# paTRICK-swk/D3DP

Measured on AMD Instinct MI355X. Metric: pose-hypotheses/sec (H x clips) at F=243, J=17, H=20, K=10, higher is better.
Workload: dtype f16x2-split operands on fp16 MFMA, f32 accumulate (fp32-class: meets 1e-3 mm)

## Files before the change

### d3dp_amd/csrc/attention_x2.hip

```cpp
#include "common.h"
#include "kernels.h"
#include "ta_common.h"
#include "attn_frag.h"

#ifndef D3DP_ATTN_OVERLAP
#define D3DP_ATTN_OVERLAP 0
#endif
#ifndef D3DP_ATTN_KPIPE
#define D3DP_ATTN_KPIPE 0
#endif
#ifndef D3DP_ATTN_MIXLO
#define D3DP_ATTN_MIXLO 0
#endif
#ifndef D3DP_ATTN_W16
#define D3DP_ATTN_W16 0
#endif
#ifndef D3DP_ATTN_STAMP
#define D3DP_ATTN_STAMP 0
#endif

namespace {

__device__ __forceinline__ f16x8 as_f16x8(bf16x8 v) { return __builtin_bit_cast(f16x8, v); }

// ... 30 lines not shown
#pragma unroll
  for (int dn = 0; dn < ND; ++dn) o[dn] = __builtin_amdgcn_mfma_f32_16x16x32_f16(vh[dn], pl[C0], o[dn], 0, 0, 0);
#pragma unroll
  for (int dn = 0; dn < ND; ++dn) o[dn] = __builtin_amdgcn_mfma_f32_16x16x32_f16(vh[dn], ph[C0], o[dn], 0, 0, 0);
  __builtin_amdgcn_sched_barrier(0);
  if constexpr (C0 + 1 < C1) pv_chunks_x2_rec<NKT, C0 + 1, C1>(fb, plane, ph, pl, o, nh, nl);
}
template <int NKT, int C0, int C1 = NKT / 2, int HD>
__device__ __forceinline__ void pv_chunks_x2(const FragBasesT<HD>& fb, int plane, const f16x8 (&ph)[NKT / 2],
                                             const f16x8 (&pl)[NKT / 2], f32x4 (&o)[HD / 16]) {
  if constexpr (C0 < C1) {
    f16x8 vh[HD / 16], vl[HD / 16];
    load_v_frags_x2<C0>(fb, plane, vh, vl);
    pv_chunks_x2_rec<NKT, C0, C1>(fb, plane, ph, pl, o, vh, vl);
  }
}

template <int C0, int HD>
__device__ __forceinline__ void pv_chunk_x2_seq(const FragBasesT<HD>& fb, int plane, const f16x8& ph, const f16x8& pl,
                                                f32x4 (&o)[HD / 16]) {
#pragma unroll
  for (int dn = 0; dn < HD / 16; ++dn) {
    const f16x8 vh = load_vt_frag<C0, f16, HD>(fb.v[dn]);
    const f16x8 vl = load_vt_frag<C0, f16, HD>(fb.v[dn] + plane);
    o[dn] = __builtin_amdgcn_mfma_f32_16x16x32_f16(vl, ph, o[dn], 0, 0, 0);
    o[dn] = __builtin_amdgcn_mfma_f32_16x16x32_f16(vh, pl, o[dn], 0, 0, 0);
    o[dn] = __builtin_amdgcn_mfma_f32_16x16x32_f16(vh, ph, o[dn], 0, 0, 0);
  }
}

// ... 74 lines not shown
  asm volatile("global_load_dwordx4 %0, %1, off" : "=v"(r) : "v"(p) : "memory");
  return r;
}
__device__ __forceinline__ void settle(f32x4& r) { asm volatile("" : "+v"(r)); }
__device__ __forceinline__ void gload16_untracked_into(f32x4& r, const float* p) {
  asm volatile("global_load_dwordx4 %0, %1, off" : "+v"(r) : "v"(p) : "memory");
}

template <int V>
__device__ __forceinline__ void wait_vmcnt() { __builtin_amdgcn_s_waitcnt((V & 15) | (7 << 4) | (15 << 8) | ((V >> 4) << 14)); }

#if D3DP_ATTN_OVERLAP || D3DP_ATTN_MIXLO || D3DP_ATTN_W16
#include "attention_x2_variants.h"
#endif

template <int NKT, bool MASK_ANY_TILE>
__device__ __forceinline__ void softmax_split_x2(f32x4 (&s)[NKT], int n, int lane, f16x8 (&ph)[NKT / 2], f16x8 (&pl)[NKT / 2],
                                                 float& denom, float cexp) {
  const int fg = lane >> 4;
  if constexpr (!MASK_ANY_TILE) {
#pragma unroll
    for (int r = 0; r < 4; ++r)
      if (16 * (NKT - 1) + 4 * fg + r >= n) s[NKT - 1][r] = -INFINITY;
  } else {
#pragma unroll
    for (int t = 0; t < NKT; ++t)
#pragma unroll
      for (int r = 0; r < 4; ++r)
        if (16 * t + 4 * fg + r >= n) s[t][r] = -INFINITY;
  }
  float mx = -INFINITY;
// ... 15 lines not shown
      const float y0 = __builtin_amdgcn_exp2f(fmaf(s[t][r], cexp, nb)), y1 = __builtin_amdgcn_exp2f(fmaf(s[t][r + 1], cexp, nb));
      sum4[0] += y0;
      sum4[1] += y1;
      const f16x2v h2 = {(f16)y0, (f16)y1};
      hp[r >> 1] = __builtin_bit_cast(unsigned, h2);
      lp[r >> 1] = x2_lo_pair_mix(y0, y1, hp[r >> 1]);
    }
    using u32x4v = unsigned __attribute__((ext_vector_type(4)));
    u32x4v hv = __builtin_bit_cast(u32x4v, ph[t >> 1]), lv = __builtin_bit_cast(u32x4v, pl[t >> 1]);
    hv[(t & 1) * 2] = hp[0]; hv[(t & 1) * 2 + 1] = hp[1];
    lv[(t & 1) * 2] = lp[0]; lv[(t & 1) * 2 + 1] = lp[1];
    ph[t >> 1] = __builtin_bit_cast(f16x8, hv);
    pl[t >> 1] = __builtin_bit_cast(f16x8, lv);
  }
#else
#pragma unroll
  for (int t = 0; t < NKT; ++t) {
#pragma unroll
    for (int r = 0; r < 4; ++r) {
      const float y = __builtin_amdgcn_exp2f(fmaf(s[t][r], cexp, nb));
      sum4[r & 1] += y;
      const f16 h = (f16)y;
      ph[t >> 1][(t & 1) * 4 + r] = h;
      pl[t >> 1][(t & 1) * 4 + r] = (f16)fmaf(y, 1.0f, -(float)h);
    }
  }
#endif
  float sum = sum4[0] + sum4[1];
  sum += __shfl_xor(sum, 16, 64);
  sum += __shfl_xor(sum, 32, 64);
// ... 39 lines not shown
    b = __builtin_amdgcn_mfma_f32_16x16x32_f16(kc[1][3], qh[1], b, 0, 0, 0);
    s[t] = a; s[t + 1] = b;
    if (t + 2 < NKT) {
#pragma unroll
      for (int j = 0; j < 2; ++j) {
        kc[j][0] = kn[j][0]; kc[j][1] = kn[j][1];
        kc[j][2] = *reinterpret_cast<const f16x8*>(fb.k0 + (t + 2 + j) * 2048);
        kc[j][3] = *reinterpret_cast<const f16x8*>(fb.k1 + (t + 2 + j) * 2048);
      }
    }
    __builtin_amdgcn_sched_barrier(0);
  }
  softmax_split_x2<NKT, MASK_ANY_TILE>(s, n, lane, ph, pl, denom, cexp);
}

template <int NKT, bool MASK_ANY_TILE>
__device__ __forceinline__ void attn_scores_x2_pair(const FragBases& fb, int plane, const f16x8 (&qh)[2][2],
                                                    const f16x8 (&ql)[2][2], int n, int lane, f16x8 (&ph)[2][NKT / 2],
                                                    f16x8 (&pl)[2][NKT / 2], float (&denom)[2], float cexp) {
  f32x4 s0[NKT], s1[NKT];
  auto read_k = [&](int t, f16x8 (&k)[4]) {
    k[0] = *reinterpret_cast<const f16x8*>(fb.k0 + plane + t * 2048);
    k[1] = *reinterpret_cast<const f16x8*>(fb.k1 + plane + t * 2048);
    k[2] = *reinterpret_cast<const f16x8*>(fb.k0 + t * 2048);
    k[3] = *reinterpret_cast<const f16x8*>(fb.k1 + t * 2048);
  };
  f16x8 kc[2][4];
#define X2_PAIR_TERM(KI, Q, D)                                                                  \
    a0 = __builtin_amdgcn_mfma_f32_16x16x32_f16(kc[0][KI], Q[0][D], a0, 0, 0, 0);               \
    b0 = __builtin_amdgcn_mfma_f32_16x16x32_f16(kc[1][KI], Q[0][D], b0, 0, 0, 0);               \
    a1 = __builtin_amdgcn_mfma_f32_16x16x32_f16(kc[0][KI], Q[1][D], a1, 0, 0, 0);               \
// ... 24 lines not shown
    if (t + 2 < NKT) { read_lo(t + 2, kc[0]); read_lo(t + 3, kc[1]); }
    __builtin_amdgcn_sched_barrier(0);
#endif
    X2_PAIR_TERM(2, ql, 0)
    X2_PAIR_TERM(3, ql, 1)
    X2_PAIR_TERM(2, qh, 0)
    X2_PAIR_TERM(3, qh, 1)
#if D3DP_ATTN_KPIPE
    __builtin_amdgcn_sched_barrier(0);
    if (t + 2 < NKT) { read_hi(t + 2, kc[0]); read_hi(t + 3, kc[1]); }
    __builtin_amdgcn_sched_barrier(0);
#endif
    s0[t] = a0; s0[t + 1] = b0; s1[t] = a1; s1[t + 1] = b1;
  }
#undef X2_PAIR_TERM
  softmax_split_x2<NKT, MASK_ANY_TILE>(s0, n, lane, ph[0], pl[0], denom[0], cexp);
  softmax_split_x2<NKT, MASK_ANY_TILE>(s1, n, lane, ph[1], pl[1], denom[1], cexp);
}

template <int HD, int NKT, bool MASK_ANY_TILE>
__device__ __forceinline__ void attn_scores_x2_hd(const FragBasesT<HD>& fb, int plane, const typename X2Head<HD>::frag& qh,
                                                  const typename X2Head<HD>::frag& ql, int n, int lane, f16x8 (&ph)[NKT / 2],
                                                  f16x8 (&pl)[NKT / 2], float& denom, float cexp) {
  typedef typename X2Head<HD>::frag frag;
  constexpr int TILE = 16 * X2Head<HD>::ROWB;
  f32x4 s[NKT];
#pragma unroll
  for (int t = 0; t < NKT; ++t) {
    const frag kl = *reinterpret_cast<const frag*>(fb.k0 + plane + t * TILE);
    const frag kh = *reinterpret_cast<const frag*>(fb.k0 + t * TILE);
    s[t] = x2_tile_scores(kh, kl, qh, ql);
    if ((t & 3) == 3) __builtin_amdgcn_sched_barrier(0);
// ... 27 lines not shown
  }
  softmax_split_x2<NKT, MASK_ANY_TILE>(s0, n, lane, ph[0], pl[0], denom[0], cexp);
  softmax_split_x2<NKT, MASK_ANY_TILE>(s1, n, lane, ph[1], pl[1], denom[1], cexp);
}

#if D3DP_ATTN_STAMP
__device__ unsigned long long d3dp_attn_stamps[4 * 8 * 16 * 8];
#define ATTN_STAMP(k)                                                                                          \
  do {                                                                                                         \
    if (blockIdx.x < 4 && iter < 16 && lane == 0)                                                              \
      d3dp_attn_stamps[((blockIdx.x * 8 + wave) * 16 + iter) * 8 + (k)] = __builtin_readcyclecounter();        \
  } while (0)
#else
#define ATTN_STAMP(k) do { } while (0)
#endif
template <int NKT, int OUTS, bool MASK_ANY_TILE, int HD = 64>
__global__ __launch_bounds__(512) void attn_temporal_x2_kernel(const float* __restrict__ qkv, void* __restrict__ out_v,
                                                               SeqMap map, int C, int heads, size_t plane_elems,
                                                               int n_prob, X2Scales sc) {
  using H = X2Head<HD>;
  constexpr int NW = 8;
  constexpr int TPW = (NKT + NW - 1) / NW;
  constexpr int NK = 16 * NKT;
  constexpr int PLANE = NK * H::ROWB;
  constexpr int NPC = PLANE / 1024;
  constexpr int PER = (NPC + NW - 1) / NW;
  constexpr int ND = HD / 16;
  __shared__ __attribute__((aligned(16))) char kimg[2 * PLANE];
  __shared__ __attribute__((aligned(16))) char vimg[2 * PLANE];
  const int n = map.n_tok;
  const int tid = threadIdx.x, lane = tid & 63;
// ... 116 lines not shown
        }
      }
    } else if constexpr (TPW == 2) {
      f16x8 qh[2][2], ql[2][2];
#pragma unroll
      for (int u = 0; u < 2; ++u) {
        float4 qf[4];
#pragma unroll
        for (int i = 0; i < 4; ++i) {
          settle(qr[u][i]);
          qf[i] = make_float4(qr[u][i][0], qr[u][i][1], qr[u][i][2], qr[u][i][3]);
        }
        ta_split8(qf[0], qf[1], qh[u][0], ql[u][0], sc.q);
        ta_split8(qf[2], qf[3], qh[u][1], ql[u][1], sc.q);
      }
      attn_scores_x2_pair<NKT, MASK_ANY_TILE>(fbk, PLANE, qh, ql, n, lane, ph, pl, denom, sc.cexp);
    } else {
      denom[0] = 1.f;
      if (wave < n_qt) {
        f16x8 qh[2], ql[2];
        float4 qf[4];
#pragma unroll
        for (int i = 0; i < 4; ++i) {
          settle(qr[0][i]);
          qf[i] = make_float4(qr[0][i][0], qr[0][i][1], qr[0][i][2], qr[0][i][3]);
        }
        ta_split8(qf[0], qf[1], qh[0], ql[0], sc.q);
        ta_split8(qf[2], qf[3], qh[1], ql[1], sc.q);
        attn_scores_x2<NKT, MASK_ANY_TILE>(fbk, PLANE, qh, ql, n, lane, ph[0], pl[0], denom[0], sc.cexp);
      }
    }
// ... 14 lines not shown
    const FragBasesT<HD> fb = make_frag_bases<HD>(kimg, vimg, opaque(lane));
#if D3DP_ATTN_OVERLAP
    if constexpr (OVL) {
      f32x4 o[4];
#pragma unroll
      for (int dn = 0; dn < 4; ++dn) o[dn] = (f32x4){0.f, 0.f, 0.f, 0.f};
      float sum1[2] = {0.f, 0.f};
      x2_pv_overlap<NKT>(fb, PLANE, ph[0], pl[0], o, s1, nb1, sc.cexp, ph[1], pl[1], sum1);
      denom[1] = x2_denominator(sum1);
      const int l = opaque(lane);
      const int q = wave * 16 + (l & 15);
      if (q < n)
        store_o_x2<OUTS>(o, inv_scale / denom[0], out_v, (size_t)(tok0 + q * ts), C, head * 64 + (l >> 4) * 4, sc.oplane);
    }
#endif
#pragma unroll
    for (int u = OVL ? 1 : 0; u < TPW; ++u) {
      if (u == TPW - 1 && (has_next || HD != 64)) load_q_raw(row0_n, head_n);
      const int qt = wave + u * NW;
      if (qt < n_qt) {
        f32x4 o[ND];
#pragma unroll
        for (int dn = 0; dn < ND; ++dn) o[dn] = (f32x4){0.f, 0.f, 0.f, 0.f};
        pv_chunks_x2<NKT, 0>(fb, PLANE, ph[u], pl[u], o);
        const int l = opaque(lane);
        const int q = qt * 16 + (l & 15);
        if (q < n)
          store_o_x2<OUTS>(o, inv_scale / denom[u], out_v, (size_t)(tok0 + q * ts), C, head * HD + (l >> 4) * 4, sc.oplane);
      }
    }
    if (!has_next) break;
    asm volatile("s_waitcnt lgkmcnt(0)" ::: "memory");
// ... 279 lines not shown
  }
}

template <typename K>
int x2_resident_per_cu(K kern, int threads, int at_most) {
  int nb = 0;
  if (hipOccupancyMaxActiveBlocksPerMultiprocessor(&nb, reinterpret_cast<const void*>(kern), threads, 0) != hipSuccess) {
    (void)hipGetLastError();
    return at_most;
  }
  return nb < 1 ? 1 : nb < at_most ? nb : at_most;
}

template <int NKT, int OUTS, int HD>
int launch_temporal_x2(const void* qkv, void* out, int n_seq, SeqMap map, int C, int heads, size_t plane, X2Scales sc,
                       hipStream_t st) {
  constexpr int NK = 16 * NKT;
  const size_t lds = (size_t)NK * X2Head<HD>::ROWB * 4;
  constexpr int NW = 8;
  const bool last_only = map.n_tok > 16 * (NKT - 1);
  auto kern = last_only ? attn_temporal_x2_kernel<NKT, OUTS, false, HD> : attn_temporal_x2_kernel<NKT, OUTS, true, HD>;
  static PerDeviceOnce once[2];
  const int n_wg = once[HD == 64 || last_only].get([&](int dev) {
    int per_cu = (int)((160 * 1024) / lds) < 2048 / (NW * 64) ? (int)((160 * 1024) / lds) : 2048 / (NW * 64);
    if constexpr (HD != 64) per_cu = x2_resident_per_cu(kern, NW * 64, per_cu);
    const int cus = d3dp_cu_count(dev);
    return cus < 0 ? cus : cus * per_cu;
  });
  if (n_wg < 0) return -3;
  const int n_prob = n_seq * heads;
#if D3DP_ATTN_W16
  if constexpr (NKT == 16 && HD == 64) {
    if (map.n_tok > 16 * (NKT - 1)) {
      hipLaunchKernelGGL((attn_temporal_x2_w16_kernel<OUTS>), dim3(n_prob < n_wg ? n_prob : n_wg), dim3(1024), 0, st,
                         (const float*)qkv, out, map, C, heads, plane, n_prob, sc);
      return 0;
    }
  }
#endif
  hipLaunchKernelGGL(kern, dim3(n_prob < n_wg ? n_prob : n_wg), dim3(NW * 64), 0, st, (const float*)qkv, out, map, C,
                     heads, plane, n_prob, sc);
  return 0;
}

template <int HD>
int launch_attn_x2_hd(int act, int axis, const void* qkv, void* out, int n_seq, SeqMap map, int C, int heads, float act_scale,
                      hipStream_t st, int hd_true) {
  const size_t plane = (size_t)n_seq * map.n_tok * C;
  const int n = map.n_tok;
  const float rsq = hd_true > 0 && hd_true != HD ? (float)(1.0 / sqrt((double)hd_true))
                                                 : (HD == 64 ? 0.125f : HD == 32 ? 0.17677669529663689f : 0.25f);
  const X2Scales sc = {act_scale, rsq * 1.44269504088896340736f / (act_scale * act_scale),
                       1.0f / act_scale, act_scale};
  if (axis == 0 && n <= 32) {
    const int n_prob = n_seq * heads;
    if (act == 3) hipLaunchKernelGGL((attn_spatial_x2_kernel<2, HD>), dim3((n_prob + 3) / 4), dim3(256), 0, st, (const float*)qkv, out, n_prob, map, C, heads, plane, sc);
    else hipLaunchKernelGGL((attn_spatial_x2_kernel<0, HD>), dim3((n_prob + 3) / 4), dim3(256), 0, st, (const float*)qkv, out, n_prob, map, C, heads, plane, sc);
    return 0;
  }
  if (n > 256) {
    const int groups = ((n + 15) / 16 + 7) / 8, n_work = n_seq * heads * groups;
    static PerDeviceOnce once[2];
    const int wgs = once[act == 3].get([&](int dev) {
      const int cus = d3dp_cu_count(dev);
      int per_cu = 2;
      if constexpr (HD != 64)
        per_cu = act == 3 ? x2_resident_per_cu(attn_temporal_x2_long_kernel<2, HD>, 512, 4) : x2_resident_per_cu(attn_temporal_x2_long_kernel<0, HD>, 512, 4);
      return cus < 0 ? cus : cus * per_cu;
    });
    if (wgs < 0) return -3;
    const dim3 grid(n_work < wgs ? n_work : wgs), blk(512);
    if (act == 3) hipLaunchKernelGGL((attn_temporal_x2_long_kernel<2, HD>), grid, blk, 0, st, (const float*)qkv, out, map, C, heads, groups, n_work, sc);
    else hipLaunchKernelGGL((attn_temporal_x2_long_kernel<0, HD>), grid, blk, 0, st, (const float*)qkv, out, map, C, heads, groups, n_work, sc);
    return 0;
  }
#define X2_CASE(NKT_)                                                                                         \
  return act == 3 ? launch_temporal_x2<NKT_, 2, HD>(qkv, out, n_seq, map, C, heads, plane, sc, st)            \
                  : launch_temporal_x2<NKT_, 0, HD>(qkv, out, n_seq, map, C, heads, plane, sc, st);
  if (n <= 32) { X2_CASE(2) }
  if (n <= 64) { X2_CASE(4) }
  if (n <= 128) { X2_CASE(8) }
  X2_CASE(16)
#undef X2_CASE
}

}

void d3dp_launch_qkv_pack_x2(const float* src, void* dst, size_t T, int C, float act_scale, hipStream_t st) {
  const size_t total = T * (size_t)(3 * C / 4);
  const unsigned blocks = (unsigned)((total + 255) / 256 < 8192 ? (total + 255) / 256 : 8192);
  hipLaunchKernelGGL(qkv_pack_x2_kernel, dim3(blocks ? blocks : 1), dim3(256), 0, st, src, (char*)dst, T, C, act_scale);
}

int d3dp_launch_attn_x2(int act, int axis, const void* qkv, void* out, int n_seq, SeqMap map, int C, int heads,
                        float act_scale, hipStream_t st, int hd_true) {
  if (heads < 1 || C % heads || map.n_tok < 1 || (act != 0 && act != 3) || !(act_scale > 0.f) || hd_true < 0 || hd_true > C / heads) return -2;
  switch (C / heads) {
    case 64: return launch_attn_x2_hd<64>(act, axis, qkv, out, n_seq, map, C, heads, act_scale, st, hd_true);
    case 32: return launch_attn_x2_hd<32>(act, axis, qkv, out, n_seq, map, C, heads, act_scale, st, hd_true);
    case 16: return launch_attn_x2_hd<16>(act, axis, qkv, out, n_seq, map, C, heads, act_scale, st, hd_true);
  }
  return -2;
}

#if D3DP_ATTN_STAMP
extern "C" __attribute__((visibility("default"))) int d3dp_debug_attn_stamps(unsigned long long* dst) {
  return (int)hipMemcpyFromSymbol(dst, HIP_SYMBOL(d3dp_attn_stamps), sizeof(unsigned long long) * 4 * 8 * 16 * 8);
}
#endif
```

### d3dp_amd/csrc/capi_denoise.hip

```cpp
#include "ctx.h"

AttnRoute attn_route(int mode, int exact_impl, int hd, int frames, int joints, bool long_rows, int axis) {
  const bool fast = mode == D3DP_MODE_FAST || mode == D3DP_MODE_FAST16, exact = mode == D3DP_MODE_EXACT;
  const bool mfma = hd == 64 || (mfma_head_dim(hd) && !long_rows);
  if (exact && exact_impl == 0 && mfma && (hd != 64 || frames <= 256 || !long_rows)) return AttnRoute::X2;
  if (fast && mfma) {
    if (axis == 0 && joints <= 32) return AttnRoute::FAST_SPATIAL;
    if (axis == 0 ? !long_rows : (frames <= 256 || !long_rows)) return AttnRoute::FAST_WHOLE_SEQ;
  }
  if (axis == 1 && exact && hd == 64 && frames <= 256) return AttnRoute::F32_TEMPORAL;
  return AttnRoute::ROWS;
}

namespace {

struct InferLayout {
  size_t temb, x, y1, y, bufA, bufB, lnst, ln_rowstat, nstat, total;
  InferLayout(const d3dp_ctx* c, int B, int H) {
    const d3dp_cfg& g = c->cfg;
    const size_t Tc = (size_t)std::min(c->chunk(), B * H) * c->seq_pitch(), C = g.channels, Cp = c->cp();
    size_t off = 0;
    auto take = [&](size_t bytes) { const size_t o = off; off += align_up(bytes); return o; };
    temb = take((size_t)B * C * 4);
    x = take(Tc * C * 4);
// ... 30 lines not shown
  Scope s(c, cls, st);
  return d3dp_linear_stream_scaled(epi, A, W, bias, out, M, N, K, st, ldexpf(1.f, r_in - r_out), ldexpf(1.f, -r_out), ldexpf(1.f, r_out));
}

int attention(d3dp_ctx* c, int axis, const void* qkv, void* out, int n_bh, float s_kv, hipStream_t st, int r_qkv = 0) {
  const d3dp_cfg& g = c->cfg;
  Scope s(c, axis == 0 ? P_ATTN_S : P_ATTN_T, st);
  const int n = axis == 0 ? n_bh * g.frames : n_bh * g.joints, act = c->act(), C = c->attn_cols();
  const SeqMap map = axis == 0 ? spatial_map(g.frames, g.joints, c->seq_pitch()) : temporal_map(g.frames, g.joints, c->seq_pitch());
  if (r_qkv != 0) {
    const AttnRoute r = c->route(axis);
    if (r != AttnRoute::FAST_SPATIAL && r != AttnRoute::FAST_WHOLE_SEQ) return -2;
    return d3dp_attn_fast_scaled(r == AttnRoute::FAST_SPATIAL ? 0 : 1, qkv, out, n, map, C, g.heads, st, ldexpf(1.f, 2 * r_qkv));
  }
  switch (c->route(axis)) {
    case AttnRoute::X2: return d3dp_launch_attn_x2(3, axis, qkv, out, n, map, C, g.heads, s_kv, st, g.channels / g.heads);
    case AttnRoute::FAST_SPATIAL: return d3dp_launch_attn_spatial_bf16(qkv, out, n, map, C, g.heads, st, c->fast_f16, g.channels / g.heads);
    case AttnRoute::FAST_WHOLE_SEQ: return d3dp_launch_attn_temporal_bf16(qkv, out, n, map, C, g.heads, st, c->fast_f16, g.channels / g.heads);
    case AttnRoute::F32_TEMPORAL: return d3dp_launch_attn_temporal_f32(act, qkv, out, n, map, C, g.heads, st);
    case AttnRoute::ROWS: break;
  }
  return d3dp_launch_attn_rows(act, qkv, out, n, map, C, g.heads, st);
}

int run_block(d3dp_ctx* c, const BlockDev& w, int axis, float* x, void* y1, void* y, void* bufA, void* bufB, float* slices,
              float* rowstat, int n_bh, hipStream_t st, float* nstat = nullptr) {
  const d3dp_cfg& g = c->cfg;
  const int Tc = n_bh * c->seq_pitch(), C = g.channels, Ca = c->attn_cols();
  const float s_o = c->x2_attn() ? w.s_kv : kActScale;
  if (w.r_qkv | w.r_proj | w.r_h | w.r_fc2) {
    LAUNCH_TRY(linear_f16(c, P_QKV, EPI_BIAS, 0, w.r_qkv, bufA, w.qkv_w, w.qkv_b, bufB, Tc, 3 * Ca, C, st));
// ... 121 lines not shown
```

### d3dp_amd/csrc/capi_ops.hip

```cpp
#include "ctx.h"

extern "C" {

int d3dp_debug_train_linear(const float* A, const float* W, const float* bias, float* out, int32_t M, int32_t N, int32_t K,
                            int32_t tail, unsigned* amax_out, int32_t amax_pos, void* stream) {
  if (!A || !W || !out || M < 1 || N < 4 || N % 4 || K < 32 || K % 32) return d3dp_fail(D3DP_EINVAL, "d3dp_debug_train_linear: bad argument");
  if (tail & ~17) return d3dp_fail(D3DP_EINVAL, "d3dp_debug_train_linear: tail = %d (bit 0: remainder rows as 16 x 64 blocks, bit 4: one pass)", tail);
  const int passes = (tail & 16) ? 1 : 3;
  tail &= 1;
  hipStream_t st = (hipStream_t)stream;
  char* buf = nullptr;
  const size_t a_bytes = (size_t)M * K * 4, w_bytes = (size_t)N * K * 4;
  HIP_TRY(hipMalloc((void**)&buf, a_bytes + w_bytes + 64));
  unsigned* amax = reinterpret_cast<unsigned*>(buf + a_bytes + w_bytes);
  float* uns = reinterpret_cast<float*>(amax + 8);
  int rc = hipMemsetAsync(amax, 0, 64, st) == hipSuccess ? 0 : -3;
  if (!rc) {
    d3dp_launch_absmax(A, (size_t)M * K, amax, st);
    d3dp_launch_absmax(W, (size_t)N * K, amax + 1, st);
    d3dp_launch_split2_dyn(A, buf, M, K, K, amax, uns, st);
    d3dp_launch_split2_dyn(W, buf + a_bytes, N, K, K, amax + 1, uns + 1, st);
    rc = d3dp_launch_linear_f16x2_dyn(buf, buf + a_bytes, bias, uns, uns + 1, out, M, N, K, 1, st, amax_out, amax_pos, tail, passes);
  }
  const hipError_t e = hipStreamSynchronize(st);
// ... 79 lines not shown
                       heads > 0 ? C / heads : 0);
    if (axis == 0 && J > 256) return d3dp_fail(D3DP_ENOTSUP, "MFMA spatial attention takes up to 256 joints; J=%d", J);
    if (axis == 0) LAUNCH_TRY(d3dp_attn_fast_scaled(J <= 32 ? 0 : 1, qkv, out, n_bh * F, spatial_map(F, J), C, heads, st, ldexpf(1.f, 2 * s)));
    else LAUNCH_TRY(d3dp_attn_fast_scaled(1, qkv, out, n_bh * J, temporal_map(F, J), C, heads, st, ldexpf(1.f, 2 * s)));
    HIP_TRY(hipGetLastError());
    return D3DP_OK;
  }
  const int hd_true = (impl & 255) == 1 ? impl >> 8 : 0;
  if (hd_true) {
    impl = 1;
    const int hdp = heads > 0 && C % heads == 0 ? C / heads : 0;
    if (!act_bf16 || !((hdp == 32 && hd_true == 24) || (hdp == 64 && (hd_true == 40 || hd_true == 48 || hd_true == 56))))
      return d3dp_fail(D3DP_ENOTSUP, "impl 1 | (true head dim << 8) takes 2-byte rows of head dim 32 holding 24 or 64 holding 40 / 48 / 56; C=%d "
                                "heads=%d true head dim %d is not one", C, heads, hd_true);
  }
  if (impl == 2) {
    if (act_bf16) return d3dp_fail(D3DP_EINVAL, "split-fp16 attention takes fp32 activations");
    if (heads < 1 || C % heads || !mfma_head_dim(C / heads))
      return d3dp_fail(D3DP_ENOTSUP, "impl 2 (split-fp16 attention) takes head dims 64, 32 and 16; C=%d heads=%d is head dim %d (the row "
                                "kernel, impl 0, takes it)", C, heads, heads > 0 ? C / heads : 0);
    void* packed = nullptr;
    const size_t T = (size_t)n_bh * F * J;
    HIP_TRY(hipMallocAsync(&packed, T * 12 * (size_t)C, st));
    d3dp_launch_qkv_pack_x2((const float*)qkv, packed, T, C, kActScale, st);
    const int rc = d3dp_launch_attn_x2(0, axis, packed, out, axis == 0 ? n_bh * F : n_bh * J,
                                       axis == 0 ? spatial_map(F, J) : temporal_map(F, J), C, heads, kActScale, st);
    HIP_TRY(hipFreeAsync(packed, st));
    LAUNCH_TRY(rc);
  } else if (impl == 1 && act_bf16 && (heads < 1 || C % heads || !mfma_head_dim(C / heads))) {
    return d3dp_fail(D3DP_ENOTSUP, "impl 1 on 2-byte rows takes head dims 64, 32 and 16; C=%d heads=%d is head dim %d (the row kernel, "
                              "impl 0, takes it)", C, heads, heads > 0 ? C / heads : 0);
  } else if (axis == 0 && impl == 1) {
    if (!act_bf16) return d3dp_fail(D3DP_EINVAL, "MFMA spatial attention needs bf16 activations");
    if (J <= 32) LAUNCH_TRY(d3dp_launch_attn_spatial_bf16(qkv, out, n_bh * F, spatial_map(F, J), C, heads, st, f16, hd_true));
    else if (J > 256) return d3dp_fail(D3DP_ENOTSUP, "MFMA spatial attention takes up to 256 joints; J=%d", J);
    else LAUNCH_TRY(d3dp_launch_attn_temporal_bf16(qkv, out, n_bh * F, spatial_map(F, J), C, heads, st, f16, hd_true));
  } else if (axis == 0) LAUNCH_TRY(d3dp_launch_attn_rows(act_bf16, qkv, out, n_bh * F, spatial_map(F, J), C, heads, st));
  else if (impl == 1 && !act_bf16) {
    LAUNCH_TRY(d3dp_launch_attn_temporal_f32(0, qkv, out, n_bh * J, temporal_map(F, J), C, heads, st));
  } else if (impl == 1) {
    if (!act_bf16) return d3dp_fail(D3DP_EINVAL, "MFMA temporal attention needs bf16 activations");
// ... 23 lines not shown
```

### d3dp_amd/csrc/ctx_plan.h

```cpp
#pragma once
#include <algorithm>
#include <cstdlib>
#include <cstring>

#include "../../include/d3dp_hip.h"

int d3dp_fail(int code, const char* fmt, ...) __attribute__((format(printf, 2, 3)));

struct CtxEnv {
  const char *exact_impl = nullptr, *long_attn = nullptr, *no_fold = nullptr, *defer_norm = nullptr, *train_impl = nullptr,
             *train_overlap = nullptr, *train_gelu = nullptr, *train_wgrad = nullptr, *train_ln_operand = nullptr, *train_tail = nullptr,
             *train_attn = nullptr, *train_passes = nullptr, *fast_impl = nullptr, *fast16_range = nullptr, *x2_skew = nullptr,
             *x2_pp = nullptr, *x2_wide = nullptr, *seq_pad = nullptr, *fold_ln = nullptr, *train_long_attn = nullptr;
  static CtxEnv from_process() {
    CtxEnv e;
    e.exact_impl = getenv("D3DP_EXACT_IMPL");
    e.long_attn = getenv("D3DP_LONG_ATTN");
    e.no_fold = getenv("D3DP_NO_FOLD");
    e.defer_norm = getenv("D3DP_DEFER_NORM");
    e.train_impl = getenv("D3DP_TRAIN_IMPL");
    e.train_overlap = getenv("D3DP_TRAIN_OVERLAP");
    e.train_gelu = getenv("D3DP_TRAIN_GELU");
    e.train_wgrad = getenv("D3DP_TRAIN_WGRAD");
    e.train_ln_operand = getenv("D3DP_TRAIN_LN_OPERAND");
    e.train_tail = getenv("D3DP_TRAIN_TAIL");
    e.train_attn = getenv("D3DP_TRAIN_ATTN");
    e.train_passes = getenv("D3DP_TRAIN_PASSES");
    e.fast_impl = getenv("D3DP_FAST_IMPL");
    e.fast16_range = getenv("D3DP_FAST16_RANGE");
    e.x2_skew = getenv("D3DP_X2_SKEW");
    e.x2_pp = getenv("D3DP_X2_PP");
    e.x2_wide = getenv("D3DP_X2_WIDE");
    e.seq_pad = getenv("D3DP_SEQ_PAD");
    e.fold_ln = getenv("D3DP_FOLD_LN");
    e.train_long_attn = getenv("D3DP_TRAIN_LONG_ATTN");
    return e;
  }
};

struct CtxPlan {
  int hdp = 0;
  bool fast16_scale = false;
  int train_passes = 3;
  int exact_impl_req = 0;
  bool long_rows = false;
  bool fold = true;
  bool defer = true;
  bool train_x2 = true;
  bool train_overlap = true;
  int train_overlap_sets = 2;
  bool train_gelu_in_prep = true;
  bool train_wgrad_merged = true;
  bool train_ln_direct = true;
  bool train_tail_blocks = true;
  int train_attn_x2 = 2;
  bool train_long_attn = false;
  int skew_d = 0;
  int pingpong = 0;
  int pad_override = -1;
  bool fold_ln_on = false;
};

inline bool env_is(const char* v, const char* s) { return v && !strcmp(v, s); }
inline int env_digit(const char* v, const char* allowed, int dflt) {
  return v && v[0] && !v[1] && strchr(allowed, v[0]) ? v[0] - '0' : dflt;
}
inline bool mfma_head_dim(int hd) { return hd == 64 || hd == 32 || hd == 16; }

inline bool instantiated_width(const d3dp_cfg& g) {
  const int hd = g.channels / g.heads;
  return (g.channels == 64 || g.channels == 128 || g.channels == 256 || g.channels == 512) &&
         (hd == 8 || hd == 16 || hd == 32 || hd == 64) && g.hidden >= 64 && g.hidden % 64 == 0;
}
inline bool optin_width(int c) { return c == 192 || c == 320 || c == 384 || c == 448; }
inline int padded_head_dim(int hd) { return hd <= 32 ? 32 : 64; }
inline bool x2_optin_shape(const d3dp_cfg& g) {
  const int hd = g.channels / g.heads;
  return optin_width(g.channels) && hd % 8 == 0 && hd <= 64 && g.hidden >= 64 && g.hidden % 64 == 0;
}
inline bool fast_optin_shape(const d3dp_cfg& g) {
  const int hd = g.channels / g.heads;
// ... 79 lines not shown
                                "{64,128,256,512} with head dim in {8,16,32,64} and hidden a multiple of 64; other widths run in D3DP_MODE_EXACT / "
                                "D3DP_MODE_TRAIN (fp32 implementation)",
                  g.channels, g.heads, g.hidden);
    if (g.channels > 1024 || g.channels % 4 || hd % 4 || hd > 128 || g.hidden < 4 || g.hidden % 4)
      return d3dp_fail(D3DP_ENOTSUP, "channels=%d heads=%d hidden=%d: the fp32 implementation takes channels <= 1024, head dim a multiple of 4 up to 128 "
                                "and hidden a multiple of 4", g.channels, g.heads, g.hidden);
    const int nmax = std::max(g.frames, g.joints), cap = hd <= 16 ? 16 : hd <= 32 ? 32 : hd <= 64 ? 64 : 128;
    if (train && !train_widths && !p.train_long_attn && (nmax > 256 || (size_t)nmax * (8 * (cap + 4) + 12) > 160 * 1024))
      return d3dp_fail(D3DP_ENOTSUP, "channels=%d heads=%d frames=%d joints=%d: training at a width outside {64,128,256,512} runs the fp32 attention "
                                "backward, which holds a whole sequence in LDS (<= 256 tokens; <= 153 at head dims above 64)",
                  g.channels, g.heads, g.frames, g.joints);
  }
  const bool train_f32 = env_is(e.train_impl, "f32");
  p.fold = !(e.no_fold && e.no_fold[0] == '1');
  p.defer = !(e.defer_norm && e.defer_norm[0] == '0');
  p.train_x2 = !train_f32 && (width_inst || train_widths);
  p.train_overlap = !(e.train_overlap && e.train_overlap[0] == '0');
  p.train_overlap_sets = (e.train_overlap && e.train_overlap[0] == '1') ? 1 : 2;
  p.train_gelu_in_prep = !env_is(e.train_gelu, "pass");
  p.train_wgrad_merged = !env_is(e.train_wgrad, "each");
  p.train_ln_direct = !env_is(e.train_ln_operand, "pass");
  p.train_tail_blocks = !env_is(e.train_tail, "split");
  p.train_attn_x2 = env_is(e.train_attn, "f32") ? 0 : env_is(e.train_attn, "x2t") ? 1 : 2;
  const bool superseded = !p.train_gelu_in_prep || !p.train_wgrad_merged || !p.train_tail_blocks || !p.train_ln_direct;
  if (train && e.train_passes) {
    if (strcmp(e.train_passes, "1") && strcmp(e.train_passes, "3"))
      return d3dp_fail(D3DP_ENOTSUP, "D3DP_TRAIN_PASSES=%.32s: the values a TRAIN context takes are D3DP_TRAIN_PASSES=1 (one fp16-MFMA pass per "
                                "product of the split-fp16 training Linears) and 3 (the default)", e.train_passes);
    if (e.train_passes[0] == '1') {
      if (!train_linears_split(p, g))
// ... 29 lines not shown
```

### d3dp_amd/csrc/kernels.h

```cpp
#pragma once
#include <hip/hip_runtime.h>
#include <stdint.h>

#include <mutex>

#include "train_plan.h"

struct PerDeviceOnce {
  static constexpr int kMaxDev = 64;
  std::mutex mu;
  int val[kMaxDev] = {0};
  template <class F> int get(F&& fn) {
    int dev = 0;
    if (hipGetDevice(&dev) != hipSuccess || dev < 0 || dev >= kMaxDev) return -3;
    std::lock_guard<std::mutex> lock(mu);
    if (val[dev] <= 0) {
      const int v = fn(dev);
      if (v <= 0) return v < 0 ? v : -3;
      val[dev] = v;
    }
    return val[dev];
  }
};
inline int d3dp_cu_count(int dev) {
// ... 72 lines not shown
                           int K, hipStream_t st);

struct SeqMap { int n_tok, inner, outer_stride, inner_stride, tok_stride; };
int d3dp_launch_attn_rows(int act_bf16, const void* qkv, void* out, int n_seq, SeqMap map, int C, int heads,
                          hipStream_t st, unsigned* amax = nullptr);
int d3dp_launch_attn_temporal_f32(int act, const void* qkv, void* out, int n_seq, SeqMap map, int C, int heads,
                                  hipStream_t st);
int d3dp_launch_attn_temporal_bf16(const void* qkv, void* out, int n_seq, SeqMap map, int C, int heads,
                                   hipStream_t st, int f16 = 0, int hd_true = 0);
int d3dp_launch_attn_spatial_bf16(const void* qkv, void* out, int n_seq, SeqMap map, int C, int heads, hipStream_t st,
                                  int f16 = 0, int hd_true = 0);
int d3dp_attn_fast_padded(int axis, const void* qkv, void* out, int n_seq, SeqMap map, int C, int heads, hipStream_t st, int f16,
                          int hd_true);
int d3dp_attn_fast_scaled(int axis, const void* qkv, void* out, int n_seq, SeqMap map, int C, int heads, hipStream_t st, float emul);
int d3dp_launch_attn_x2(int act, int axis, const void* qkv, void* out, int n_seq, SeqMap map, int C, int heads,
                        float act_scale, hipStream_t st, int hd_true = 0);
void d3dp_launch_qkv_pack_x2(const float* src, void* dst, size_t T, int C, float act_scale, hipStream_t st);

int d3dp_launch_time_mlp(const int64_t* t, const float* freq, const float* w1, const float* b1, const float* w2,
                         const float* b2, float* temb, int B, int C, hipStream_t st);
int d3dp_launch_embed_ln(int act_bf16, const float* x2d, const float* x3d, const float* temb, const float* ew,
                         const float* eb, const float* spos, const float* lnw, const float* lnb, float eps, float* x,
                         void* xn, int seq0, int n_seq, int H, int F, int J, int C, hipStream_t st, int SP = 0);
int d3dp_launch_ln(int act_bf16, float* x, const void* yadd, int write_x, const float* w, const float* b, float eps,
                   void* xn, int T, int C, hipStream_t st);
int d3dp_launch_ln2(int act_bf16, float* x, const void* yadd0, const void* yadd, const float* wa, const float* ba, const float* pos,
                    const float* wb, const float* bb, float eps, void* xn, int T, int C, int F, int J, hipStream_t st,
                    int SP = 0);
int d3dp_launch_ln2_defer(int act_bf16, const float* x, const float* wa, const float* ba, const float* wb, const float* bb, float eps,
                          void* xn, float* stat, int T, int C, hipStream_t st);
int d3dp_rows2_embed_ln(int act, const float* x2d, const float* x3d, const float* temb, const float* ew, const float* eb,
// ... 103 lines not shown
```

Baseline: 51.21.

## Share V fragments across two query tiles in temporal x2 attention PV

Adds a VSHARE path for the temporal split-fp16 attention kernel (HD=64, NKT=16). It computes PV for both of a wave's query tiles at once, in two head-dim halves, so each loaded V fragment feeds MFMAs for both tiles instead of being reloaded per tile. It also adds a v_fma_mix based computation of the low-half softmax residual. The path is on by default and can be turned off with an env var; it costs extra template instantiations and higher accumulator register pressure in the shared loop.

```diff
diff --git a/d3dp_amd/csrc/attention_x2.hip b/d3dp_amd/csrc/attention_x2.hip
--- a/d3dp_amd/csrc/attention_x2.hip
+++ b/d3dp_amd/csrc/attention_x2.hip
@@ -68,6 +68,44 @@
     load_v_frags_x2<C0>(fb, plane, vh, vl);
     pv_chunks_x2_rec<NKT, C0, C1>(fb, plane, ph, pl, o, vh, vl);
   }
+}
+
+template <int C0, int DN0>
+__device__ __forceinline__ void load_v_frags_x2_half(const FragBases& fb, int plane, f16x8 (&vh)[2], f16x8 (&vl)[2]) {
+#pragma unroll
+  for (int d = 0; d < 2; ++d) {
+    vh[d] = load_vt_frag<C0, f16, 64>(fb.v[DN0 + d]);
+    vl[d] = load_vt_frag<C0, f16, 64>(fb.v[DN0 + d] + plane);
+  }
+}
+template <int NKT, int DN0, int C0>
+__device__ __forceinline__ void pv_half_x2_rec(const FragBases& fb, int plane, const f16x8 (&ph)[2][NKT / 2],
+                                               const f16x8 (&pl)[2][NKT / 2], f32x4 (&o)[2][2], const f16x8 (&vh)[2],
+                                               const f16x8 (&vl)[2]) {
+  f16x8 nh[2], nl[2];
+  if constexpr (C0 + 1 < NKT / 2) load_v_frags_x2_half<C0 + 1, DN0>(fb, plane, nh, nl);
+  __builtin_amdgcn_sched_barrier(0);
+#pragma unroll
+  for (int d = 0; d < 2; ++d)
+#pragma unroll
+    for (int u = 0; u < 2; ++u) o[u][d] = __builtin_amdgcn_mfma_f32_16x16x32_f16(vl[d], ph[u][C0], o[u][d], 0, 0, 0);
+#pragma unroll
+  for (int d = 0; d < 2; ++d)
+#pragma unroll
+    for (int u = 0; u < 2; ++u) o[u][d] = __builtin_amdgcn_mfma_f32_16x16x32_f16(vh[d], pl[u][C0], o[u][d], 0, 0, 0);
+#pragma unroll
+  for (int d = 0; d < 2; ++d)
+#pragma unroll
+    for (int u = 0; u < 2; ++u) o[u][d] = __builtin_amdgcn_mfma_f32_16x16x32_f16(vh[d], ph[u][C0], o[u][d], 0, 0, 0);
+  __builtin_amdgcn_sched_barrier(0);
+  if constexpr (C0 + 1 < NKT / 2) pv_half_x2_rec<NKT, DN0, C0 + 1>(fb, plane, ph, pl, o, nh, nl);
+}
+template <int NKT, int DN0>
+__device__ __forceinline__ void pv_half_x2(const FragBases& fb, int plane, const f16x8 (&ph)[2][NKT / 2],
+                                           const f16x8 (&pl)[2][NKT / 2], f32x4 (&o)[2][2]) {
+  f16x8 vh[2], vl[2];
+  load_v_frags_x2_half<0, DN0>(fb, plane, vh, vl);
+  pv_half_x2_rec<NKT, DN0, 0>(fb, plane, ph, pl, o, vh, vl);
 }
 
 template <int C0, int HD>
@@ -172,7 +210,17 @@
 #include "attention_x2_variants.h"
 #endif
 
-template <int NKT, bool MASK_ANY_TILE>
+__device__ __forceinline__ unsigned x2_lo_pair_f32mix(float y0, float y1, unsigned hp) {
+  unsigned lp;
+  float t;
+  asm("v_fma_mix_f32 %0, %2, 1.0, -%4 op_sel_hi:[0,0,1]\n\t"
+      "v_fma_mix_f32 %1, %3, 1.0, -%4 op_sel:[0,0,1] op_sel_hi:[0,0,1]\n\t"
+      "v_cvt_pk_f16_f32 %0, %0, %1"
+      : "=&v"(lp), "=&v"(t) : "v"(y0), "v"(y1), "v"(hp));
+  return lp;
+}
+
+template <int NKT, bool MASK_ANY_TILE, bool LO_MIX = false>
 __device__ __forceinline__ void softmax_split_x2(f32x4 (&s)[NKT], int n, int lane, f16x8 (&ph)[NKT / 2], f16x8 (&pl)[NKT / 2],
                                                  float& denom, float cexp) {
   const int fg = lane >> 4;
@@ -218,6 +266,28 @@
     pl[t >> 1] = __builtin_bit_cast(f16x8, lv);
   }
 #else
+  if constexpr (LO_MIX) {
+    using f16x2v = _Float16 __attribute__((ext_vector_type(2)));
+    using f32x2v = float __attribute__((ext_vector_type(2)));
+    using u32x4v = unsigned __attribute__((ext_vector_type(4)));
+#pragma unroll
+    for (int t = 0; t < NKT; ++t) {
+      unsigned hp[2], lp[2];
+#pragma unroll
+      for (int r = 0; r < 4; r += 2) {
+        const float y0 = __builtin_amdgcn_exp2f(fmaf(s[t][r], cexp, nb)), y1 = __builtin_amdgcn_exp2f(fmaf(s[t][r + 1], cexp, nb));
+        sum4[0] += y0;
+        sum4[1] += y1;
+        hp[r >> 1] = __builtin_bit_cast(unsigned, __builtin_convertvector((f32x2v){y0, y1}, f16x2v));
+        lp[r >> 1] = x2_lo_pair_f32mix(y0, y1, hp[r >> 1]);
+      }
+      u32x4v hv = __builtin_bit_cast(u32x4v, ph[t >> 1]), lv = __builtin_bit_cast(u32x4v, pl[t >> 1]);
+      hv[(t & 1) * 2] = hp[0]; hv[(t & 1) * 2 + 1] = hp[1];
+      lv[(t & 1) * 2] = lp[0]; lv[(t & 1) * 2 + 1] = lp[1];
+      ph[t >> 1] = __builtin_bit_cast(f16x8, hv);
+      pl[t >> 1] = __builtin_bit_cast(f16x8, lv);
+    }
+  } else
 #pragma unroll
   for (int t = 0; t < NKT; ++t) {
 #pragma unroll
@@ -287,7 +357,7 @@
   softmax_split_x2<NKT, MASK_ANY_TILE>(s, n, lane, ph, pl, denom, cexp);
 }
 
-template <int NKT, bool MASK_ANY_TILE>
+template <int NKT, bool MASK_ANY_TILE, bool LO_MIX = false>
 __device__ __forceinline__ void attn_scores_x2_pair(const FragBases& fb, int plane, const f16x8 (&qh)[2][2],
                                                     const f16x8 (&ql)[2][2], int n, int lane, f16x8 (&ph)[2][NKT / 2],
                                                     f16x8 (&pl)[2][NKT / 2], float (&denom)[2], float cexp) {
@@ -342,8 +412,8 @@
     s0[t] = a0; s0[t + 1] = b0; s1[t] = a1; s1[t + 1] = b1;
   }
 #undef X2_PAIR_TERM
-  softmax_split_x2<NKT, MASK_ANY_TILE>(s0, n, lane, ph[0], pl[0], denom[0], cexp);
-  softmax_split_x2<NKT, MASK_ANY_TILE>(s1, n, lane, ph[1], pl[1], denom[1], cexp);
+  softmax_split_x2<NKT, MASK_ANY_TILE, LO_MIX>(s0, n, lane, ph[0], pl[0], denom[0], cexp);
+  softmax_split_x2<NKT, MASK_ANY_TILE, LO_MIX>(s1, n, lane, ph[1], pl[1], denom[1], cexp);
 }
 
 template <int HD, int NKT, bool MASK_ANY_TILE>
@@ -401,7 +471,7 @@
 #else
 #define ATTN_STAMP(k) do { } while (0)
 #endif
-template <int NKT, int OUTS, bool MASK_ANY_TILE, int HD = 64>
+template <int NKT, int OUTS, bool MASK_ANY_TILE, int HD = 64, bool VSHARE = false>
 __global__ __launch_bounds__(512) void attn_temporal_x2_kernel(const float* __restrict__ qkv, void* __restrict__ out_v,
                                                                SeqMap map, int C, int heads, size_t plane_elems,
                                                                int n_prob, X2Scales sc) {
@@ -548,7 +618,7 @@
         ta_split8(qf[0], qf[1], qh[u][0], ql[u][0], sc.q);
         ta_split8(qf[2], qf[3], qh[u][1], ql[u][1], sc.q);
       }
-      attn_scores_x2_pair<NKT, MASK_ANY_TILE>(fbk, PLANE, qh, ql, n, lane, ph, pl, denom, sc.cexp);
+      attn_scores_x2_pair<NKT, MASK_ANY_TILE, VSHARE && !D3DP_ATTN_MIXLO>(fbk, PLANE, qh, ql, n, lane, ph, pl, denom, sc.cexp);
     } else {
       denom[0] = 1.f;
       if (wave < n_qt) {
@@ -593,8 +663,30 @@
         store_o_x2<OUTS>(o, inv_scale / denom[0], out_v, (size_t)(tok0 + q * ts), C, head * 64 + (l >> 4) * 4, sc.oplane);
     }
 #endif
-#pragma unroll
-    for (int u = OVL ? 1 : 0; u < TPW; ++u) {
+    constexpr bool SHARE = VSHARE && HD == 64 && TPW == 2 && !OVL;
+    if constexpr (SHARE) {
+      const int l = opaque(lane);
+      const int q0 = wave * 16 + (l & 15);
+      const bool tile1 = wave + NW < n_qt;
+      const float inv[2] = {inv_scale / denom[0], inv_scale / denom[1]};
+#pragma unroll
+      for (int half = 0; half < 2; ++half) {
+        if (half == 1 && has_next) load_q_raw(row0_n, head_n);
+        f32x4 o[2][2];
+#pragma unroll
+        for (int u = 0; u < 2; ++u)
+#pragma unroll
+          for (int d = 0; d < 2; ++d) o[u][d] = (f32x4){0.f, 0.f, 0.f, 0.f};
+        if (half == 0) pv_half_x2<NKT, 0>(fb, PLANE, ph, pl, o);
+        else pv_half_x2<NKT, 2>(fb, PLANE, ph, pl, o);
+        const int col = head * 64 + half * 32 + (l >> 4) * 4;
+        if (q0 < n) store_o_x2<OUTS>(o[0], inv[0], out_v, (size_t)(tok0 + q0 * ts), C, col, sc.oplane);
+        if (tile1 && q0 + 16 * NW < n)
+          store_o_x2<OUTS>(o[1], inv[1], out_v, (size_t)(tok0 + (q0 + 16 * NW) * ts), C, col, sc.oplane);
+      }
+    }
+#pragma unroll
+    for (int u = (OVL ? 1 : 0) + (SHARE ? TPW : 0); u < TPW; ++u) {
       if (u == TPW - 1 && (has_next || HD != 64)) load_q_raw(row0_n, head_n);
       const int qt = wave + u * NW;
       if (qt < n_qt) {
@@ -904,12 +996,15 @@
 
 template <int NKT, int OUTS, int HD>
 int launch_temporal_x2(const void* qkv, void* out, int n_seq, SeqMap map, int C, int heads, size_t plane, X2Scales sc,
-                       hipStream_t st) {
+                       hipStream_t st, bool vshare) {
   constexpr int NK = 16 * NKT;
   const size_t lds = (size_t)NK * X2Head<HD>::ROWB * 4;
   constexpr int NW = 8;
   const bool last_only = map.n_tok > 16 * (NKT - 1);
   auto kern = last_only ? attn_temporal_x2_kernel<NKT, OUTS, false, HD> : attn_temporal_x2_kernel<NKT, OUTS, true, HD>;
+  if constexpr (HD == 64 && NKT == 16 && !(D3DP_ATTN_OVERLAP || D3DP_ATTN_KPIPE || D3DP_ATTN_MIXLO || D3DP_ATTN_W16)) {
+    if (vshare) kern = last_only ? attn_temporal_x2_kernel<NKT, OUTS, false, HD, true> : attn_temporal_x2_kernel<NKT, OUTS, true, HD, true>;
+  }
   static PerDeviceOnce once[2];
   const int n_wg = once[HD == 64 || last_only].get([&](int dev) {
     int per_cu = (int)((160 * 1024) / lds) < 2048 / (NW * 64) ? (int)((160 * 1024) / lds) : 2048 / (NW * 64);
@@ -935,7 +1030,7 @@
 
 template <int HD>
 int launch_attn_x2_hd(int act, int axis, const void* qkv, void* out, int n_seq, SeqMap map, int C, int heads, float act_scale,
-                      hipStream_t st, int hd_true) {
+                      hipStream_t st, int hd_true, bool vshare) {
   const size_t plane = (size_t)n_seq * map.n_tok * C;
   const int n = map.n_tok;
   const float rsq = hd_true > 0 && hd_true != HD ? (float)(1.0 / sqrt((double)hd_true))
@@ -965,8 +1060,8 @@
     return 0;
   }
 #define X2_CASE(NKT_)                                                                                         \
-  return act == 3 ? launch_temporal_x2<NKT_, 2, HD>(qkv, out, n_seq, map, C, heads, plane, sc, st)            \
-                  : launch_temporal_x2<NKT_, 0, HD>(qkv, out, n_seq, map, C, heads, plane, sc, st);
+  return act == 3 ? launch_temporal_x2<NKT_, 2, HD>(qkv, out, n_seq, map, C, heads, plane, sc, st, vshare)    \
+                  : launch_temporal_x2<NKT_, 0, HD>(qkv, out, n_seq, map, C, heads, plane, sc, st, vshare);
   if (n <= 32) { X2_CASE(2) }
   if (n <= 64) { X2_CASE(4) }
   if (n <= 128) { X2_CASE(8) }
@@ -983,12 +1078,12 @@
 }
 
 int d3dp_launch_attn_x2(int act, int axis, const void* qkv, void* out, int n_seq, SeqMap map, int C, int heads,
-                        float act_scale, hipStream_t st, int hd_true) {
+                        float act_scale, hipStream_t st, int hd_true, bool vshare) {
   if (heads < 1 || C % heads || map.n_tok < 1 || (act != 0 && act != 3) || !(act_scale > 0.f) || hd_true < 0 || hd_true > C / heads) return -2;
   switch (C / heads) {
-    case 64: return launch_attn_x2_hd<64>(act, axis, qkv, out, n_seq, map, C, heads, act_scale, st, hd_true);
-    case 32: return launch_attn_x2_hd<32>(act, axis, qkv, out, n_seq, map, C, heads, act_scale, st, hd_true);
-    case 16: return launch_attn_x2_hd<16>(act, axis, qkv, out, n_seq, map, C, heads, act_scale, st, hd_true);
+    case 64: return launch_attn_x2_hd<64>(act, axis, qkv, out, n_seq, map, C, heads, act_scale, st, hd_true, vshare);
+    case 32: return launch_attn_x2_hd<32>(act, axis, qkv, out, n_seq, map, C, heads, act_scale, st, hd_true, vshare);
+    case 16: return launch_attn_x2_hd<16>(act, axis, qkv, out, n_seq, map, C, heads, act_scale, st, hd_true, vshare);
   }
   return -2;
 }
diff --git a/d3dp_amd/csrc/capi_denoise.hip b/d3dp_amd/csrc/capi_denoise.hip
--- a/d3dp_amd/csrc/capi_denoise.hip
+++ b/d3dp_amd/csrc/capi_denoise.hip
@@ -68,7 +68,7 @@
     return d3dp_attn_fast_scaled(r == AttnRoute::FAST_SPATIAL ? 0 : 1, qkv, out, n, map, C, g.heads, st, ldexpf(1.f, 2 * r_qkv));
   }
   switch (c->route(axis)) {
-    case AttnRoute::X2: return d3dp_launch_attn_x2(3, axis, qkv, out, n, map, C, g.heads, s_kv, st, g.channels / g.heads);
+    case AttnRoute::X2: return d3dp_launch_attn_x2(3, axis, qkv, out, n, map, C, g.heads, s_kv, st, g.channels / g.heads, c->attn_vshare);
     case AttnRoute::FAST_SPATIAL: return d3dp_launch_attn_spatial_bf16(qkv, out, n, map, C, g.heads, st, c->fast_f16, g.channels / g.heads);
     case AttnRoute::FAST_WHOLE_SEQ: return d3dp_launch_attn_temporal_bf16(qkv, out, n, map, C, g.heads, st, c->fast_f16, g.channels / g.heads);
     case AttnRoute::F32_TEMPORAL: return d3dp_launch_attn_temporal_f32(act, qkv, out, n, map, C, g.heads, st);
diff --git a/d3dp_amd/csrc/capi_ops.hip b/d3dp_amd/csrc/capi_ops.hip
--- a/d3dp_amd/csrc/capi_ops.hip
+++ b/d3dp_amd/csrc/capi_ops.hip
@@ -117,6 +117,8 @@
       return d3dp_fail(D3DP_ENOTSUP, "impl 1 | (true head dim << 8) takes 2-byte rows of head dim 32 holding 24 or 64 holding 40 / 48 / 56; C=%d "
                                 "heads=%d true head dim %d is not one", C, heads, hd_true);
   }
+  const int x2_planes = impl == (2 | (1 << 8));
+  if (x2_planes) impl = 2;
   if (impl == 2) {
     if (act_bf16) return d3dp_fail(D3DP_EINVAL, "split-fp16 attention takes fp32 activations");
     if (heads < 1 || C % heads || !mfma_head_dim(C / heads))
@@ -126,8 +128,9 @@
     const size_t T = (size_t)n_bh * F * J;
     HIP_TRY(hipMallocAsync(&packed, T * 12 * (size_t)C, st));
     d3dp_launch_qkv_pack_x2((const float*)qkv, packed, T, C, kActScale, st);
-    const int rc = d3dp_launch_attn_x2(0, axis, packed, out, axis == 0 ? n_bh * F : n_bh * J,
-                                       axis == 0 ? spatial_map(F, J) : temporal_map(F, J), C, heads, kActScale, st);
+    const int rc = d3dp_launch_attn_x2(x2_planes ? 3 : 0, axis, packed, out, axis == 0 ? n_bh * F : n_bh * J,
+                                       axis == 0 ? spatial_map(F, J) : temporal_map(F, J), C, heads, kActScale, st, 0,
+                                       attn_vshare_on(getenv("D3DP_ATTN_VSHARE")));
     HIP_TRY(hipFreeAsync(packed, st));
     LAUNCH_TRY(rc);
   } else if (impl == 1 && act_bf16 && (heads < 1 || C % heads || !mfma_head_dim(C / heads))) {
diff --git a/d3dp_amd/csrc/ctx_plan.h b/d3dp_amd/csrc/ctx_plan.h
--- a/d3dp_amd/csrc/ctx_plan.h
+++ b/d3dp_amd/csrc/ctx_plan.h
@@ -11,13 +11,14 @@
   const char *exact_impl = nullptr, *long_attn = nullptr, *no_fold = nullptr, *defer_norm = nullptr, *train_impl = nullptr,
              *train_overlap = nullptr, *train_gelu = nullptr, *train_wgrad = nullptr, *train_ln_operand = nullptr, *train_tail = nullptr,
              *train_attn = nullptr, *train_passes = nullptr, *fast_impl = nullptr, *fast16_range = nullptr, *x2_skew = nullptr,
-             *x2_pp = nullptr, *x2_wide = nullptr, *seq_pad = nullptr, *fold_ln = nullptr, *train_long_attn = nullptr;
+             *x2_pp = nullptr, *x2_wide = nullptr, *seq_pad = nullptr, *fold_ln = nullptr, *train_long_attn = nullptr, *attn_vshare = nullptr;
   static CtxEnv from_process() {
     CtxEnv e;
     e.exact_impl = getenv("D3DP_EXACT_IMPL");
     e.long_attn = getenv("D3DP_LONG_ATTN");
     e.no_fold = getenv("D3DP_NO_FOLD");
     e.defer_norm = getenv("D3DP_DEFER_NORM");
+    e.attn_vshare = getenv("D3DP_ATTN_VSHARE");
     e.train_impl = getenv("D3DP_TRAIN_IMPL");
     e.train_overlap = getenv("D3DP_TRAIN_OVERLAP");
     e.train_gelu = getenv("D3DP_TRAIN_GELU");
@@ -46,6 +47,7 @@
   bool long_rows = false;
   bool fold = true;
   bool defer = true;
+  bool attn_vshare = true;
   bool train_x2 = true;
   bool train_overlap = true;
   int train_overlap_sets = 2;
@@ -65,6 +67,7 @@
 inline int env_digit(const char* v, const char* allowed, int dflt) {
   return v && v[0] && !v[1] && strchr(allowed, v[0]) ? v[0] - '0' : dflt;
 }
+inline bool attn_vshare_on(const char* v) { return !(v && v[0] == '0'); }
 inline bool mfma_head_dim(int hd) { return hd == 64 || hd == 32 || hd == 16; }
 
 inline bool instantiated_width(const d3dp_cfg& g) {
@@ -174,6 +177,7 @@
   const bool train_f32 = env_is(e.train_impl, "f32");
   p.fold = !(e.no_fold && e.no_fold[0] == '1');
   p.defer = !(e.defer_norm && e.defer_norm[0] == '0');
+  p.attn_vshare = attn_vshare_on(e.attn_vshare);
   p.train_x2 = !train_f32 && (width_inst || train_widths);
   p.train_overlap = !(e.train_overlap && e.train_overlap[0] == '0');
   p.train_overlap_sets = (e.train_overlap && e.train_overlap[0] == '1') ? 1 : 2;
diff --git a/d3dp_amd/csrc/kernels.h b/d3dp_amd/csrc/kernels.h
--- a/d3dp_amd/csrc/kernels.h
+++ b/d3dp_amd/csrc/kernels.h
@@ -110,7 +110,7 @@
                           int hd_true);
 int d3dp_attn_fast_scaled(int axis, const void* qkv, void* out, int n_seq, SeqMap map, int C, int heads, hipStream_t st, float emul);
 int d3dp_launch_attn_x2(int act, int axis, const void* qkv, void* out, int n_seq, SeqMap map, int C, int heads,
-                        float act_scale, hipStream_t st, int hd_true = 0);
+                        float act_scale, hipStream_t st, int hd_true = 0, bool vshare = true);
 void d3dp_launch_qkv_pack_x2(const float* src, void* dst, size_t T, int C, float act_scale, hipStream_t st);
 
 int d3dp_launch_time_mlp(const int64_t* t, const float* freq, const float* w1, const float* b1, const float* w2,
```

Result: no change. 51.44 (median of 6 runs) (+0.5%).
